# Kyo-suke-S/Depth_image_captioning_pub

Measured on AMD Instinct MI355X. Metric: images/sec (train, depth-soft, 224x224, seq-len 20), higher is better.
Workload: dtype f32; 1 GPU; depth-soft train step, synthetic RGB-D 224x224, batch 64/GPU, seq-len 20, V=10000, ResNet-152 (random init, batch-stat BN) + depth CNN + soft-attention LSTM; global_batch=64, batch_per_gpu=64, seq_len=20, vocab=10000, parallelism=dp1, resnet_conv_mode=f16x2, cross_step_resnet_overlap=True, resnet_forwards_in_flight=3, annotation_cells=49, ranks=1, collective=none (single rank)

## Files before the change

depth_image_captioning_pub_amd/csrc/api.hip:

```cpp
#include "dic.h"
#include "conv.h"
#include "nn_kernels.h"

#include <cstdio>

using namespace dic;

namespace dic { void resnet_fuse_bn_operand(int mask); void resnet_fuse_bn_halo(int on); void resnet_fuse_res_bn(int on); void depth_encoder_l1_sparse(int on); void bn_finalize_two_level_rows(int rows); void resnet_debug_fused_tail_bn(int on); void conv1_depth_debug_blocks(int n);
                void depth_encoder_f16x2(int on); }
#ifdef DIC_EXPERIMENTS
namespace dic { void decoder_debug_persistent(int on); void decoder_persist_debug_buffer(unsigned long long* p); void decoder_persist_debug_placement(int p);
                void resnet_debug_skip_bn_apply(int on); }
#endif

extern "C" {

int dic_version(void) { return DIC_ABI_VERSION; }
size_t dic_struct_bytes(int which) {
  switch (which) {
    case 0: return sizeof(dic_conv_bn_layer);
    case 1: return sizeof(dic_decoder_weights);
    case 2: return sizeof(dic_decoder_grads);
    case 3: return sizeof(dic_depth_encoder_weights);
    case 4: return sizeof(dic_depth_encoder_grads);
    case 5: return sizeof(dic_depth_bn_state);
    case 6: return sizeof(dic_nic_weights);
    case 7: return sizeof(dic_nic_grads);
    default: return 0;
  }
}
const char* dic_last_error(void) { return last_error(); }

int dic_gemm_f32(int M, int N, int K, const float* A, long long lda, int a_colk, const float* B, long long ldb,
                 int b_colk, float* C, long long ldc, const float* bias, int act, int accumulate, int splitk,
                 float* workspace, size_t workspace_bytes, int force_tile, void* stream) {
  GemmParams p{};
  p.M = M; p.N = N; p.K = K;
  p.A = a_colk ? op_colk(A, lda) : op_rowk(A, lda);
  p.B = b_colk ? op_colk(B, ldb) : op_rowk(B, ldb);
  p.ep = ep_store(C, ldc, bias, act);
  p.ep.accumulate = accumulate;
  p.splitk = splitk; p.ws = workspace;
  p.ablate = force_tile / 1000;
  force_tile %= 1000;
  DIC_REQUIRE(force_tile == 0 || force_tile == 64 || force_tile == 128, "force_tile must be 0, 64 or 128");
  if (splitk > 1)
    DIC_REQUIRE(workspace_bytes >= gemm_splitk_ws_bytes(M, N, splitk), "dic_gemm_f32: workspace too small");
  return gemm_launch(p, (hipStream_t)stream, force_tile);
}

int dic_conv2d_fwd(const float* x, int B, int H, int W, int C, int in_nchw, const float* w_ohwi, const float* bias,
                   int CO, int KH, int KW, int stride, int pad, float* y_nhwc, float* bn_partial, int* mtiles_out,
                   int force_tile, float* tail_ws, void* stream) {
  ConvDesc d{B, H, W, C, CO, KH, KW, stride, pad, in_nchw};
  return conv_fwd(x, d, w_ohwi, bias, y_nhwc, bn_partial, mtiles_out, (hipStream_t)stream, force_tile, tail_ws);
}

int dic_debug_force_staged_gemm(int on) {
  if (gemm_bf3_force_tile(on) == 0) return 0;
  if (on >= 100 && on <= 104) { dic::resnet_fuse_bn_operand(on == 104 ? -1 : on - 100); return 0; }
  if (on == 98 || on == 99) { dic::resnet_fuse_res_bn(on - 98); return 0; }
  if (on == 108 || on == 109) { dic::resnet_fuse_bn_halo(on - 108); return 0; }
  if (on == 182 || on == 183) { dic::bn_finalize_two_level_rows(on == 182 ? 512 : 1024); return 0; }
  if (on == 180 || on == 181) { dic::depth_encoder_l1_sparse(on - 180); return 0; }
  if (on == 116 || on == 117) { dic::depth_encoder_f16x2(on - 116); return 0; }
#ifdef DIC_EXPERIMENTS
  if (on == 140 || on == 141) { dic::decoder_debug_persistent(on - 140); return 0; }
  if (on == 142 || on == 143) { dic::decoder_persist_debug_placement(on - 142); return 0; }
  if (on >= 130 && on <= 134) { dic::conv1_depth_debug_blocks(256 * (on - 130)); return 0; }
  if (on >= 150 && on <= 153) { dic::resnet_debug_fused_tail_bn(on - 150); return 0; }
  if (on >= 124 && on <= 127) { dic::resnet_debug_skip_bn_apply(on == 125 ? 3 : on == 126 ? 2 : on == 127 ? 1 : 0); return 0; }
  if (on >= 0 && on <= 13) { gemm_force_v1(on); return 0; }
#endif
  DIC_REQUIRE(false, "debug switch: unknown code %d", on);
  return 0;
}
#ifdef DIC_EXPERIMENTS
int dic_debug_decoder_stamps(unsigned long long* dev_buf) { dic::decoder_persist_debug_buffer(dev_buf); return 0; }
#endif
int dic_debug_conv1_wgrad(const float* x, int B, int H, int W, const float* dy, float* dw, float* dbias, float* ws, float* cs_ws,
                          void* stream) {
  ConvDesc d{B, H, W, 1, 128, 7, 7, 3, 0, 0};
  return conv1_depth_wgrad(x, d, dy, dw, dbias, ws, cs_ws, (hipStream_t)stream);
}
int dic_debug_conv1_fwd(const float* x, int B, int H, int W, const float* w, const float* bias, float* y, float* partial,
                        void* stream) {
  ConvDesc d{B, H, W, 1, 128, 7, 7, 3, 0, 0};
  int rows = 0;
  return conv1_depth_fwd(x, d, w, bias, y, partial, &rows, (hipStream_t)stream);
}
int dic_debug_conv_bf3(const uint16_t* const x_planes[3], int B, int H, int W, int C, const uint16_t* const w_planes[3], int CO,
                       int k, int stride, int pad, float* y, float* bn_partial, int* mtiles_out, float* tail_ws, void* stream) {
  ConvDesc d{B, H, W, C, CO, k, k, stride, pad, 0};
  return conv_fwd_bf3(x_planes, d, w_planes, y, bn_partial, mtiles_out, tail_ws, (hipStream_t)stream, nullptr, nullptr, nullptr);
}
// ... 350 lines not shown
```

depth_image_captioning_pub_amd/csrc/conv.h:

```cpp
#pragma once
#include "gemm.h"

namespace dic {

struct ConvDesc {
  int B, H, W, C;
  int CO, KH, KW, stride, pad;
  int in_nchw;
  int OH() const { return (H + 2 * pad - KH) / stride + 1; }
  int OW() const { return (W + 2 * pad - KW) / stride + 1; }
  int M() const { return B * OH() * OW(); }
  int K() const { return KH * KW * C; }
  ConvGeom geom() const { return ConvGeom{H, W, C, OH(), OW(), KH, KW, stride, pad, in_nchw}; }
};

int conv_fwd(const float* x, const ConvDesc& d, const float* w_ohwi, const float* bias, float* y,
             float* bn_partial, int* mtiles_out, hipStream_t st, int force_tile = 0, float* tail_ws = nullptr);
int conv_mtiles(const ConvDesc& d, int force_tile = 0);

int conv_fwd_bf3(const unsigned short* const x_planes[3], const ConvDesc& d, const unsigned short* const w_planes[3],
                 float* y, float* bn_partial, int* mtiles_out, float* tail_ws, hipStream_t st,
                 const float* bias = nullptr, const BnFuseArgs* bn_fuse = nullptr, int* bn_fused = nullptr,
                 int act = 0 , int tail_ws_slabs = 256 ,
                 int fmt = 0 ,
                 float out_scale = 1.0f ,
                 const float* alpha_dev0 = nullptr, const float* alpha_dev1 = nullptr );
int conv1x1_fwd_bf3_bn(const float* raw, const float* scale, const float* shift, const float* res, int relu, float* act_out,
                       int M, int C, const unsigned short* const w_planes[3], int CO, float* y, float* bn_partial,
                       int* mtiles_out, float* tail_ws, int tail_ws_slabs, hipStream_t st, const BnFuseArgs* bn_fuse = nullptr,
                       int* bn_fused = nullptr, int fmt = 0, float out_scale = 1.0f,
                       unsigned* status = nullptr ,
                       const float* res_scale = nullptr, const float* res_shift = nullptr );
bool conv1x1_bf3_bn_eligible(const float* raw, int M, int C, int CO, float* tail_ws, int tail_ws_slabs, int fmt = 0);
int bf3_plan_route(int route, int fmt, const ConvDesc& d, int flags, int splitk, int tail_ws_slabs, const char** kernel, int out[6]);
int conv3x3_fwd_bf3_bn(const float* raw, const float* scale, const float* shift, int relu, const ConvDesc& d,
                       const unsigned short* const w_planes[3], float* y, float* bn_partial, int* mtiles_out, float* tail_ws,
                       int tail_ws_slabs, hipStream_t st, const BnFuseArgs* bn_fuse, int* bn_fused, int fmt, float out_scale, unsigned* status);
#ifdef DIC_EXPERIMENTS
bool conv1x1_astat_eligible(int M, int C, int CO);
int conv1x1_astat_bn(const float* raw, const float* scale, const float* shift, int relu, int M, int C, const unsigned short* const w_planes[3],
                     int CO, float* y, float* bn_partial, int* mtiles_out, hipStream_t st, float out_scale, unsigned* status = nullptr);
#endif
constexpr int kResnetTailSlabs = 1024;
size_t conv_wgrad_bf3_plane_elems(const ConvDesc& d, int which);
size_t conv_wgrad_bf3_ws_floats(const ConvDesc& d, int splitk);
int conv_wgrad_bf3(const float* x, const ConvDesc& d, const float* dy, float* dw_ohwi, int splitk,
                   unsigned short* const dyT[3], unsigned short* const pT[3], float* ws, hipStream_t st,
                   int fmt = 0, const float* dy_slot = nullptr );
size_t conv_stem_bf3_plane_elems(int B, int H, int W);
int conv_stem_pack_weights(const float* w_oihw, int CO, float* scratch_f32, unsigned short* const w_planes[3], hipStream_t st,
                           float f16_scale = 0.f );
int conv_stem_bf3(const float* imgs_nchw, int B, int H, int W, int CO, unsigned short* const x_planes[3],
                  const unsigned short* const w_planes[3], float* y, float* bn_partial, int* mtiles_out, hipStream_t st,
                  int fmt = 0, float out_scale = 1.0f, unsigned* status = nullptr );
int conv_dgrad_s1_bf3(const unsigned short* const dy_planes[3], const ConvDesc& d,
                      const unsigned short* const wflip_planes[3], float* dx, hipStream_t st, float* tail_ws = nullptr,
                      int tail_ws_slabs = 256, int fmt = 0, const float* alpha_dev0 = nullptr, const float* alpha_dev1 = nullptr);
int split_bf16x3(const float* x, long long n, unsigned short* hi, unsigned short* mid, unsigned short* lo, hipStream_t st);
int split_bf16x3_paired(const float* x, long long rows, int K, unsigned short* hi, unsigned short* mid,
                        unsigned short* lo, hipStream_t st);
int split_f16x2_paired(const float* x, long long rows, int K, float scale, unsigned short* h1, unsigned short* h2, hipStream_t st,
                       unsigned* status = nullptr );

int conv1_depth_fwd(const float* x, const ConvDesc& d, const float* w, const float* bias, float* y, float* bn_partial,
                    int* partial_rows, hipStream_t st);
int conv1_depth_fwd_blocks(const ConvDesc& d);
bool conv1_depth_supported(const ConvDesc& d);
size_t conv1_depth_wgrad_ws_floats(const ConvDesc& d);
struct BnBuf;
bool depth_layer1_sparse_supported(const ConvDesc& d);
size_t depth_layer1_sparse_ws_floats(const ConvDesc& d);
int conv1_depth_wgrad(const float* x, const ConvDesc& d, const float* dy, float* dw, float* dbias, float* ws, float* cs_ws,
                      hipStream_t st);
int depth_layer1_backward_sparse(const float* depth, const ConvDesc& d, const float* dpool, const unsigned char* idx, const float* xsel,
                                 const float* conv_w, const float* conv_b, const float* gamma, BnBuf bn, float* dgamma, float* dbeta,
                                 float* dW, float* db, float* bn_ws, float* ws, float* cs_ws, hipStream_t st);
int depth_prepare_weights(const float* w2, const float* w3, unsigned short* const w2_pl[3], unsigned short* const w2f_pl[3],
                          unsigned short* const w3_pl[3], unsigned short* const w3f_pl[3], const float* slots, hipStream_t st);
int conv_wgrad(const float* x, const ConvDesc& d, const float* dy, float* dw_ohwi, int splitk, float* ws,
               hipStream_t st);
int conv_dgrad_s1(const float* dy, const ConvDesc& d, const float* w_flip, float* dx, hipStream_t st);
int conv_flip_weights(const float* w_ohwi, const ConvDesc& d, float* w_flip, hipStream_t st);

}
```

depth_image_captioning_pub_amd/csrc/encoders.hip:

```cpp
#include "dic.h"
#include "conv.h"
#include "nn_kernels.h"
#include <algorithm>
#include <vector>

namespace dic {

struct DepthGeom {
  int B, H, W;
  int H1, W1, P1h, P1w, H2, W2, P2h, P2w;
  ConvDesc c1, c2, c3;
  long long M1, M2, M3;
};

static DepthGeom depth_geom(int B, int H, int W) {
  DepthGeom g{};
  g.B = B; g.H = H; g.W = W;
  g.c1 = ConvDesc{B, H, W, 1, 128, 7, 7, 3, 0, 1};
  g.H1 = g.c1.OH(); g.W1 = g.c1.OW();
  g.P1h = g.H1 / 3; g.P1w = g.W1 / 3;
  g.c2 = ConvDesc{B, g.P1h, g.P1w, 128, 512, 3, 3, 1, 0, 0};
  g.H2 = g.c2.OH(); g.W2 = g.c2.OW();
  g.P2h = g.H2 / 3; g.P2w = g.W2 / 3;
  g.c3 = ConvDesc{B, g.P2h, g.P2w, 512, 2048, 1, 1, 1, 0, 0};
// ... 224 lines not shown
                      (double)d.M(), kBnEps, kBnMomentum, fmt ? ws.status : nullptr};
  const int rc = conv1x1_fwd_bf3_bn(raw, in_bn.scale, in_bn.shift, res, 1, act_out, d.M(), d.C, wp, d.CO, y, train_bn ? ws.partial : nullptr,
                                    &mtiles, ws.tail, kResnetTailSlabs, st, (train_bn && g_fused_tail_bn) ? &fa : nullptr, &fused, fmt,
                                    fmt ? 1.0f / (kF16ActScale * L.w_scale) : 1.0f, fmt ? ws.status : nullptr,
                                    res_bn ? res_bn->scale : nullptr, res_bn ? res_bn->shift : nullptr);
  if (rc != DIC_OK) return rc;
  if (train_bn && fused) return DIC_OK;
  if (train_bn)
    return bn_finalize_train(ws.partial, mtiles, d.M(), d.CO, L.gamma, L.beta, L.running_mean, L.running_var, bn, ws.red, st,
                             fmt ? ws.status : nullptr);
  return bn_finalize_eval(d.CO, L.gamma, L.beta, L.running_mean, L.running_var, bn, st);
}

#ifdef DIC_EXPERIMENTS
static int conv_bn_bf3_astat(const float* raw, const BnBuf& in_bn, const ConvDesc& d, const dic_conv_bn_layer& L, float* y, const RnWs& ws,
                             int train_bn, hipStream_t st, const BnBuf& bn) {
  if (!(d.KH == 1 && d.KW == 1 && d.stride == 1 && d.pad == 0) || !conv1x1_astat_eligible(d.M(), d.C, d.CO)) return 1;
  int mtiles = 0;
  const unsigned short* wp[3] = {L.w_hi, L.w_mid, nullptr};
  DIC_TRY(conv1x1_astat_bn(raw, in_bn.scale, in_bn.shift, 1, d.M(), d.C, wp, d.CO, y, train_bn ? ws.partial : nullptr, &mtiles, st,
                           1.0f / (kF16ActScale * L.w_scale), ws.status));
  if (train_bn)
    return bn_finalize_train(ws.partial, mtiles, d.M(), d.CO, L.gamma, L.beta, L.running_mean, L.running_var, bn, ws.red, st, ws.status);
  return bn_finalize_eval(d.CO, L.gamma, L.beta, L.running_mean, L.running_var, bn, st);
}
#endif

static int g_fuse_bn_operand_switch = -1;
void resnet_fuse_bn_operand(int mask) { g_fuse_bn_operand_switch = mask < 0 ? -1 : (mask & 3); }
static int g_fuse_res_bn = 1;
void resnet_fuse_res_bn(int on) { g_fuse_res_bn = on; }
static int g_fuse_bn_halo = 1;
void resnet_fuse_bn_halo(int on) { g_fuse_bn_halo = on; }

static int conv_bn_bf3_halo_fused(const float* raw, const BnBuf& in_bn, const ConvDesc& d, const dic_conv_bn_layer& L, float* y, const RnWs& ws,
                                  int train_bn, hipStream_t st, const BnBuf& bn, int fmt) {
  if (!fmt || !g_fuse_bn_halo) return 1;
  int mtiles = 0, fused = 0;
  const unsigned short* wp[3] = {L.w_hi, L.w_mid, L.w_lo};
  const BnFuseArgs fa{L.gamma, L.beta, L.running_mean, L.running_var, bn.scale, bn.shift, bn.mean, bn.invstd,
                      (double)d.M(), kBnEps, kBnMomentum, ws.status};
  const int rc = conv3x3_fwd_bf3_bn(raw, in_bn.scale, in_bn.shift, 1, d, wp, y, train_bn ? ws.partial : nullptr, &mtiles, ws.tail, kResnetTailSlabs, st,
                                    (train_bn && g_fused_tail_bn) ? &fa : nullptr, &fused, fmt, 1.0f / (kF16ActScale * L.w_scale), ws.status);
  if (rc != DIC_OK) return rc;
  if (train_bn && fused) return DIC_OK;
  if (train_bn)
    return bn_finalize_train(ws.partial, mtiles, d.M(), d.CO, L.gamma, L.beta, L.running_mean, L.running_var, bn, ws.red, st, ws.status);
  return bn_finalize_eval(d.CO, L.gamma, L.beta, L.running_mean, L.running_var, bn, st);
}

static int resnet_fwd_bf3(const dic_conv_bn_layer* layers, const int* blocks, const float* imgs_nchw, int B, int train_bn,
                          float* features, const RnPlan& pl, const RnWs& ws, hipStream_t st, int pool_out, int fmt) {
  const int g_fuse_bn_operand = g_fuse_bn_operand_switch >= 0 ? g_fuse_bn_operand_switch : (fmt ? 1 : 3);
  unsigned* const guard = fmt ? ws.status : nullptr;
  size_t ci = 0;
  float *R2 = ws.act[0], *R3 = ws.act[1], *R1 = ws.act[2], *Cf = ws.act[3];
  float* const IN[2] = {ws.act[4], ws.act[5]};
  float* const X = ws.act[0];
  unsigned short* pset[3][3];
  for (int i = 0; i < 3; ++i)
    for (int j = 0; j < 3; ++j) pset[i][j] = (fmt && j == 2) ? nullptr : ws.planes[i][j];
  unsigned short* const* Xp = pset[0];
  unsigned short* const* P1 = pset[1];
  unsigned short* const* P2 = pset[2];
  {
    const RnConv& c = pl.convs[ci++];
    const dic_conv_bn_layer& L0 = layers[c.layer];
    const bool stem_f16 = fmt && L0.w_hi && L0.w_mid && !L0.w_lo && L0.w_scale > 0.f;
    if (g_strip_stem && L0.w_hi && L0.w_mid && (L0.w_lo || stem_f16) && c.d.H % 2 == 0 && c.d.W % 2 == 0) {
      int mtiles = 0;
      const unsigned short* wp[3] = {L0.w_hi, L0.w_mid, L0.w_lo};
      DIC_TRY(conv_stem_bf3(imgs_nchw, B, c.d.H, c.d.W, 64, ws.stem_planes, wp, R3, train_bn ? ws.partial : nullptr, &mtiles, st,
                            stem_f16 ? 1 : 0, stem_f16 ? 1.0f / (kF16ActScale * L0.w_scale) : 1.0f, guard));
      if (train_bn)
        DIC_TRY(bn_finalize_train(ws.partial, mtiles, c.d.M(), 64, L0.gamma, L0.beta, L0.running_mean, L0.running_var, ws.bn,
                                  ws.red, st, guard));
      else
        DIC_TRY(bn_finalize_eval(64, L0.gamma, L0.beta, L0.running_mean, L0.running_var, ws.bn, st));
    } else
    DIC_TRY(conv_bn(imgs_nchw, c.d, layers[c.layer], R3, ws.partial, ws.bn, ws.red, ws.tail, train_bn, st));
    DIC_TRY(bn_relu_maxpool(R3, B, c.d.OH(), c.d.OW(), 64, &ws.bn, 1, 3, 2, 1, nullptr, nullptr, st, Xp, guard));
  }
  for (int s = 0; s < 4; ++s) {
    bool pending = false;
    const float* pend_res = nullptr;
    const BnBuf* pend_res_bn = nullptr;
    const float* in32_carry = nullptr;
    for (int b = 0; b < blocks[s]; ++b) {
      const RnConv& c1 = pl.convs[ci++];
      const RnConv& c2 = pl.convs[ci++];
      const RnConv& c3 = pl.convs[ci++];
      const float* in32 = in32_carry;
      in32_carry = nullptr;
      if (pending) {
        float* in_b = IN[b & 1];
        int rc = conv_bn_bf3_fused(R3, ws.bn3, pend_res, in_b, c1.d, layers[c1.layer], R1, ws, train_bn, st, ws.bn, fmt, pend_res_bn);
        if (rc == 1) {
          DIC_BN_APPLY_PLANES_OUT(R3, pend_res, nullptr, in_b, Xp, c1.d.M(), c1.d.C, ws.bn3, 1, st, pend_res_bn, guard);
          rc = conv_bn_bf3(Xp, c1.d, layers[c1.layer], R1, ws, train_bn, st, nullptr, fmt);
        }
        DIC_TRY(rc);
        in32 = in_b;
      } else {
        DIC_TRY(conv_bn_bf3(Xp, c1.d, layers[c1.layer], R1, ws, train_bn, st, nullptr, fmt));
      }
      {
        int rc = conv_bn_bf3_halo_fused(R1, ws.bn, c2.d, layers[c2.layer], R2, ws, train_bn, st, ws.bn2, fmt);
        if (rc == 1) {
          DIC_BN_APPLY_PLANES(R1, nullptr, nullptr, nullptr, P1, c1.d.M(), c1.d.CO, ws.bn, 1, st, nullptr, guard);
          rc = conv_bn_bf3(P1, c2.d, layers[c2.layer], R2, ws, train_bn, st, &ws.bn2, fmt);
        }
        DIC_TRY(rc);
      }
      if (b == 0) {
// ... 234 lines not shown

int dic_depth_encoder_bwd_map(const dic_depth_encoder_weights* w, const float* depth, const float* d_feature_map, int B,
                              int H, int W, const dic_depth_encoder_grads* gr, void* workspace, size_t workspace_bytes,
                              void* stream) {
  return depth_encoder_bwd_impl(w, depth, d_feature_map, B, H, W, gr, workspace, workspace_bytes, stream, 0);
}

int dic_depth_encoder_inspect(const void* workspace, size_t workspace_bytes, int B, int H, int W, int which, void* out,
                              long long* n_out, void* stream) {
  DIC_REQUIRE(workspace && B > 0 && which >= 1 && which <= 5, "depth_encoder_inspect: bad arguments");
  const DepthGeom g = depth_geom(B, H, W);
  bool ov = false;
  DepthWs ws = depth_carve(const_cast<void*>(workspace), workspace_bytes, g, &ov);
  DIC_REQUIRE(!ov, "depth_encoder_inspect: workspace too small");
  const long long n = which <= 2 ? (long long)B * g.P1h * g.P1w * 128
                      : which <= 4 ? (long long)B * g.P2h * g.P2w * 512 : g.M3 * 2048;
  if (n_out) *n_out = n;
  if (!out) return DIC_OK;
  if (which == 5) return relu_mask_export(ws.x3, g.M3, 2048, ws.bn3, (unsigned char*)out, (hipStream_t)stream);
  const void* src = which == 1 ? (const void*)ws.y1p : which == 2 ? (const void*)ws.idx1 : which == 3 ? (const void*)ws.y2p
                                                                                                      : (const void*)ws.idx2;
  const size_t bytes = (size_t)n * ((which & 1) ? sizeof(float) : 1);
  DIC_CHECK_HIP(hipMemcpyAsync(out, src, bytes, hipMemcpyDeviceToDevice, (hipStream_t)stream));
  return DIC_OK;
}

int dic_resnet_pack_stem_weights(const float* w_oihw, float* scratch_f32, uint16_t* w_hi, uint16_t* w_mid, uint16_t* w_lo,
                                 void* stream) {
  DIC_REQUIRE(w_oihw && scratch_f32 && w_hi && w_mid && w_lo, "resnet_pack_stem_weights: null pointer");
  unsigned short* wp[3] = {w_hi, w_mid, w_lo};
  return conv_stem_pack_weights(w_oihw, 64, scratch_f32, wp, (hipStream_t)stream);
}

int dic_resnet_pack_stem_weights_f16x2(const float* w_oihw, float* scratch_f32, uint16_t* w_h1, uint16_t* w_h2, float w_scale, void* stream) {
  DIC_REQUIRE(w_oihw && scratch_f32 && w_h1 && w_h2 && w_scale > 0.f, "resnet_pack_stem_weights_f16x2: null pointer / scale");
  unsigned short* wp[3] = {w_h1, w_h2, nullptr};
  return conv_stem_pack_weights(w_oihw, 64, scratch_f32, wp, (hipStream_t)stream, w_scale);
}

int dic_resnet_num_layers(const int* blocks) {
  int n = 1;
  for (int s = 0; s < 4; ++s) n += 3 * blocks[s] + 1;
  return n;
}

size_t dic_resnet_workspace_bytes(int B, int H, int W, const int* blocks, int mode) {
  bool ov;
  return rn_carve(nullptr, 0, resnet_plan(B, H, W, blocks), mode, &ov).bytes;
}

static int resnet_fwd_impl(const dic_conv_bn_layer* layers, int n_layers, const int* blocks, const float* imgs_nchw, int B,
                           int H, int W, int train_bn, int mode, float* features, void* workspace, size_t workspace_bytes,
                           void* stream, int pool_out) {
  hipStream_t st = (hipStream_t)stream;
  DIC_REQUIRE(layers && blocks && imgs_nchw && features && workspace, "resnet_fwd: null pointer");
  DIC_REQUIRE(n_layers == dic_resnet_num_layers(blocks), "resnet_fwd: expected %d conv+bn layers, got %d",
              dic_resnet_num_layers(blocks), n_layers);
  DIC_REQUIRE(B > 0 && H >= 32 && W >= 32, "resnet_fwd: bad input size");
  const RnPlan pl = resnet_plan(B, H, W, blocks);
  bool ov = false;
  DIC_REQUIRE(mode >= 0 && mode <= 2, "resnet_fwd: mode must be 0 (exact-fp32 MFMA), 1 (bf16x3 split MFMA) or 2 (f16x2 split MFMA)");
  RnWs ws = rn_carve(workspace, workspace_bytes, pl, mode, &ov);
  DIC_REQUIRE(!ov, "resnet_fwd: workspace too small (%zu < %zu)", workspace_bytes, ws.bytes);
  DIC_TRY(clear_status(ws.status, st));
  if (mode >= 1) {
    for (int i = 1; i < n_layers; ++i) {
// ... 58 lines not shown
```

include/dic.h:

```cpp
#ifndef DIC_H_
#define DIC_H_
#include <stddef.h>
#include <stdint.h>

#ifdef __cplusplus
extern "C" {
#endif

#define DIC_L 196
#define DIC_D 2048
#define DIC_A 128
#define DIC_E 128
#define DIC_H 128

#define DIC_ABI_VERSION 200
int dic_version(void);
const char* dic_last_error(void);
size_t dic_struct_bytes(int which);

int dic_gemm_f32(int M, int N, int K, const float* A, long long lda, int a_colk, const float* B, long long ldb,
                 int b_colk, float* C, long long ldc, const float* bias, int act, int accumulate, int splitk,
                 float* workspace, size_t workspace_bytes, int force_tile, void* stream);

int dic_conv2d_fwd(const float* x, int B, int H, int W, int C, int in_nchw, const float* w_ohwi, const float* bias,
// ... 328 lines not shown
                     float out_scale, void* stream);
int dic_gemm_bf16x3(int M, int N, int K, const uint16_t* a_hi, const uint16_t* a_mid, const uint16_t* a_lo,
                    long long lda, const uint16_t* b_hi, const uint16_t* b_mid, const uint16_t* b_lo, long long ldb,
                    float* C, long long ldc, const float* bias, void* stream);

int dic_weight_standardize(const float* w, int O, int K, float eps, float* out, void* stream);
int dic_pad_nhwc(const float* x, int B, int H, int W, int C, int top, int left, int bottom, int right, float value,
                 float* out, void* stream);
int dic_maxpool_nhwc(const float* x, int B, int H, int W, int C, int k, int stride, float* out, void* stream);
size_t dic_groupnorm_workspace_bytes(int B, int groups);
int dic_groupnorm_nhwc(const float* x, int B, long long HW, int C, int groups, const float* gamma, const float* beta,
                       float eps, const float* residual, int relu, float* out, void* workspace, void* stream);
int dic_layernorm(const float* x, long long rows, int C, const float* gamma, const float* beta, float eps, float* out,
                  void* stream);
size_t dic_vit_attention_workspace_bytes(int B, int N, int heads);
int dic_vit_attention(const float* qkv, int B, int N, int heads, int head_dim, float* out, void* workspace,
                      size_t workspace_bytes, void* stream);
int dic_upsample2x_bilinear_nhwc(const float* x, int B, int H, int W, int C, float* out, void* stream);
int dic_add_act(const float* a, const float* b, long long n, long long period, int act, float* out, void* stream);
int dic_pointwise_dot(const float* x, long long rows, int C, const float* w, const float* bias, int relu, float* out,
                      void* stream);

int dic_normalize_images(const float* in, float* out, int B, int C, int H, int W, const float* mean3, const float* std3,
                         void* stream);
int dic_resize_bilinear(const float* in, int planes, int H, int W, int resize_short, int crop, float mul, float add,
                        float* out, void* stream);
int dic_depth_standardize(float* depth, int B, long long hw, void* stream);
int dic_bn_ema_update(float* running, const float* delta, long long n, float momentum, void* stream);
int dic_bn_ema_update_guarded(float* running, const float* delta, long long n, float momentum, const uint32_t* skip_if_raised,
                              void* stream);
int dic_gather_rows(const float* table, const int64_t* idx, int n, long long row_floats, float* out, void* stream);

int dic_debug_force_staged_gemm(int on);
int dic_debug_bn_finalize(const float* partial, int mtiles, long long count, int C, const float* gamma, const float* beta,
                          float* running_mean, float* running_var, float* scale, float* shift, float* mean, float* invstd, double* red,
                          size_t red_doubles, uint32_t* status, void* stream);
int dic_debug_bn_finalize_eval(int C, const float* gamma, const float* beta, const float* running_mean, const float* running_var,
                               float* scale, float* shift, float* mean, float* invstd, void* stream);
int dic_debug_bn_apply(const float* x, const float* residual, const uint16_t* const residual_planes[3], float* y, uint16_t* const planes[3],
                       long long rows, int C, const float* scale, const float* shift, const float* mean, const float* invstd, int relu,
                       const float* res_scale, const float* res_shift, const float* res_mean, const float* res_invstd, uint32_t* status,
                       void* stream);
int dic_debug_bn_relu_maxpool(const float* x, int B, int H, int W, int C, const float* scale, const float* shift, const float* mean,
                              const float* invstd, int relu, int k, int s, int p, float* y, unsigned char* idx, uint16_t* const planes[3],
                              uint32_t* status, float* xsel, void* stream);
int dic_debug_adaptive_avgpool(const float* x, int B, int H, int W, int C, const float* scale, const float* shift, const float* mean,
                               const float* invstd, int relu, int out, float* y, void* stream);
int dic_debug_adaptive_avgpool_bwd(const float* dy, int B, int H, int W, int C, int out, float* dx, void* stream);
int dic_debug_maxpool_relu_bwd(const float* dpool, const unsigned char* idx, const float* x, int B, int H, int W, int C, int k,
                               const float* scale, const float* shift, const float* mean, const float* invstd, float* dy, void* stream);
int dic_debug_relu_mask_bwd(float* dy, const float* x, long long rows, int C, const float* scale, const float* shift, const float* mean,
                            const float* invstd, void* stream);
int dic_debug_bn_backward_ws_floats(int C);
int dic_debug_bn_backward(float* dy_dx, const float* x, long long rows, int C, const float* gamma, const float* scale, const float* shift,
                          const float* mean, const float* invstd, float* dgamma, float* dbeta, float* ws, size_t ws_floats,
                          uint16_t* const dx_planes[3], uint32_t* f16_bound, float* f16_slot, void* stream);
int dic_debug_bn_pool_backward(const float* dpool, const unsigned char* idx, const float* x, int B, int H, int W, int C, int k,
                               const float* gamma, const float* scale, const float* shift, const float* mean, const float* invstd,
                               float* dgamma, float* dbeta, float* ws, size_t ws_floats, float* dy, uint16_t* const dy_planes[3],
                               uint32_t* f16_bound, float* f16_slot, void* stream);
int dic_debug_colsum_rows(const float* X, long long ld, long long rows, int C, float* out, float* ws, size_t ws_floats, void* stream);
int dic_debug_f16_scale_reset(uint32_t* bounds, int n, void* stream);
int dic_debug_f16_scale_from_absmax(const float* x, long long n, uint32_t* bound, float* slot, void* stream);
int dic_debug_f16_scale_finish(uint32_t* bound, float* slot, void* stream);
int dic_debug_conv_wgrad_sizes(int B, int H, int W, int C, int CO, int k, int stride, int pad, int splitk, size_t* dyT_elems, size_t* pT_elems,
                               size_t* ws_floats);
// ... 31 lines not shown
```

Baseline: 7540 images/s.

## Fuse ResNet stem conv with maxpool via pooled max/min and deferred BN

Adds a fused stem kernel that computes the 7x7 stride-2 conv with f16x2 MFMA per pooled tile, accumulates the BN statistics, and writes only the 3x3 maxpool max and min of the raw conv output instead of the full 112x112x64 map. A second pass applies BN+ReLU and chooses max or min according to the sign of the BN scale, which keeps the result exact. This removes the write and re-read of the large stem activation and the separate bn_relu_maxpool pass. In exchange, pooling windows overlap across tiles, so some conv outputs are recomputed at tile halos, and the new path is enabled by default.

```diff
diff --git a/depth_image_captioning_pub_amd/csrc/api.hip b/depth_image_captioning_pub_amd/csrc/api.hip
--- a/depth_image_captioning_pub_amd/csrc/api.hip
+++ b/depth_image_captioning_pub_amd/csrc/api.hip
@@ -6,7 +6,7 @@
 
 using namespace dic;
 
-namespace dic { void resnet_fuse_bn_operand(int mask); void resnet_fuse_bn_halo(int on); void resnet_fuse_res_bn(int on); void depth_encoder_l1_sparse(int on); void bn_finalize_two_level_rows(int rows); void resnet_debug_fused_tail_bn(int on); void conv1_depth_debug_blocks(int n);
+namespace dic { void resnet_fuse_bn_operand(int mask); void resnet_fuse_bn_halo(int on); void resnet_fuse_res_bn(int on); void resnet_stem_fused(int on); void depth_encoder_l1_sparse(int on); void bn_finalize_two_level_rows(int rows); void resnet_debug_fused_tail_bn(int on); void conv1_depth_debug_blocks(int n);
                 void depth_encoder_f16x2(int on); }
 #ifdef DIC_EXPERIMENTS
 namespace dic { void decoder_debug_persistent(int on); void decoder_persist_debug_buffer(unsigned long long* p); void decoder_persist_debug_placement(int p);
@@ -61,6 +61,7 @@
   if (on >= 100 && on <= 104) { dic::resnet_fuse_bn_operand(on == 104 ? -1 : on - 100); return 0; }
   if (on == 98 || on == 99) { dic::resnet_fuse_res_bn(on - 98); return 0; }
   if (on == 108 || on == 109) { dic::resnet_fuse_bn_halo(on - 108); return 0; }
+  if (on == 186 || on == 187) { dic::resnet_stem_fused(on - 186); return 0; }
   if (on == 182 || on == 183) { dic::bn_finalize_two_level_rows(on == 182 ? 512 : 1024); return 0; }
   if (on == 180 || on == 181) { dic::depth_encoder_l1_sparse(on - 180); return 0; }
   if (on == 116 || on == 117) { dic::depth_encoder_f16x2(on - 116); return 0; }
diff --git a/depth_image_captioning_pub_amd/csrc/conv.h b/depth_image_captioning_pub_amd/csrc/conv.h
--- a/depth_image_captioning_pub_amd/csrc/conv.h
+++ b/depth_image_captioning_pub_amd/csrc/conv.h
@@ -53,6 +53,12 @@
 int conv_stem_bf3(const float* imgs_nchw, int B, int H, int W, int CO, unsigned short* const x_planes[3],
                   const unsigned short* const w_planes[3], float* y, float* bn_partial, int* mtiles_out, hipStream_t st,
                   int fmt = 0, float out_scale = 1.0f, unsigned* status = nullptr );
+struct BnBuf;
+int conv_stem_pool_rows(int B, int H, int W);
+int conv_stem_pool_f16(const float* imgs_nchw, int B, int H, int W, const unsigned short* w_h1, const unsigned short* w_h2, float out_scale,
+                       float* pmax, float* pmin, float* bn_partial, unsigned* status, hipStream_t st);
+int stem_pool_bn_relu(const float* pmax, const float* pmin, long long rows, const BnBuf& bn, float* y, unsigned short* const planes[3],
+                      unsigned* status, hipStream_t st);
 int conv_dgrad_s1_bf3(const unsigned short* const dy_planes[3], const ConvDesc& d,
                       const unsigned short* const wflip_planes[3], float* dx, hipStream_t st, float* tail_ws = nullptr,
                       int tail_ws_slabs = 256, int fmt = 0, const float* alpha_dev0 = nullptr, const float* alpha_dev1 = nullptr);
@@ -67,7 +73,6 @@
 int conv1_depth_fwd_blocks(const ConvDesc& d);
 bool conv1_depth_supported(const ConvDesc& d);
 size_t conv1_depth_wgrad_ws_floats(const ConvDesc& d);
-struct BnBuf;
 bool depth_layer1_sparse_supported(const ConvDesc& d);
 size_t depth_layer1_sparse_ws_floats(const ConvDesc& d);
 int conv1_depth_wgrad(const float* x, const ConvDesc& d, const float* dy, float* dw, float* dbias, float* ws, float* cs_ws,
diff --git a/depth_image_captioning_pub_amd/csrc/encoders.hip b/depth_image_captioning_pub_amd/csrc/encoders.hip
--- a/depth_image_captioning_pub_amd/csrc/encoders.hip
+++ b/depth_image_captioning_pub_amd/csrc/encoders.hip
@@ -280,6 +280,27 @@
 void resnet_fuse_res_bn(int on) { g_fuse_res_bn = on; }
 static int g_fuse_bn_halo = 1;
 void resnet_fuse_bn_halo(int on) { g_fuse_bn_halo = on; }
+static int g_stem_fused = 1;
+void resnet_stem_fused(int on) { g_stem_fused = on; }
+
+static bool stem_fused_takes(int B, int H, int W) {
+  return g_stem_fused && H % 2 == 0 && W % 2 == 0 && H >= 6 && W >= 6 &&
+         conv_stem_pool_rows(B, H, W) <= (int)((long long)B * (H / 2) * (W / 2) / 32 + 4);
+}
+static int stem_fused_fwd(const float* imgs_nchw, int B, int H, int W, const dic_conv_bn_layer& L0, int train_bn, float* mm, float* partial,
+                          double* red, const BnBuf& bn, float* y, unsigned short* const planes[3], unsigned* guard, hipStream_t st) {
+  const int OH = H / 2, OW = W / 2, PH = (OH - 1) / 2 + 1, PW = (OW - 1) / 2 + 1;
+  const long long rows = (long long)B * PH * PW;
+  float *pmax = mm, *pmin = mm + rows * 64;
+  DIC_TRY(conv_stem_pool_f16(imgs_nchw, B, H, W, L0.w_hi, L0.w_mid, 1.0f / (kF16ActScale * L0.w_scale), pmax, pmin,
+                             train_bn ? partial : nullptr, guard, st));
+  if (train_bn)
+    DIC_TRY(bn_finalize_train(partial, conv_stem_pool_rows(B, H, W), (long long)B * OH * OW, 64, L0.gamma, L0.beta, L0.running_mean,
+                              L0.running_var, bn, red, st, guard));
+  else
+    DIC_TRY(bn_finalize_eval(64, L0.gamma, L0.beta, L0.running_mean, L0.running_var, bn, st));
+  return stem_pool_bn_relu(pmax, pmin, rows, bn, y, planes, guard, st);
+}
 
 static int conv_bn_bf3_halo_fused(const float* raw, const BnBuf& in_bn, const ConvDesc& d, const dic_conv_bn_layer& L, float* y, const RnWs& ws,
                                   int train_bn, hipStream_t st, const BnBuf& bn, int fmt) {
@@ -315,6 +336,9 @@
     const RnConv& c = pl.convs[ci++];
     const dic_conv_bn_layer& L0 = layers[c.layer];
     const bool stem_f16 = fmt && L0.w_hi && L0.w_mid && !L0.w_lo && L0.w_scale > 0.f;
+    if (stem_f16 && g_strip_stem && stem_fused_takes(B, c.d.H, c.d.W)) {
+      DIC_TRY(stem_fused_fwd(imgs_nchw, B, c.d.H, c.d.W, L0, train_bn, R3, ws.partial, ws.red, ws.bn, nullptr, Xp, guard, st));
+    } else {
     if (g_strip_stem && L0.w_hi && L0.w_mid && (L0.w_lo || stem_f16) && c.d.H % 2 == 0 && c.d.W % 2 == 0) {
       int mtiles = 0;
       const unsigned short* wp[3] = {L0.w_hi, L0.w_mid, L0.w_lo};
@@ -328,6 +352,7 @@
     } else
     DIC_TRY(conv_bn(imgs_nchw, c.d, layers[c.layer], R3, ws.partial, ws.bn, ws.red, ws.tail, train_bn, st));
     DIC_TRY(bn_relu_maxpool(R3, B, c.d.OH(), c.d.OW(), 64, &ws.bn, 1, 3, 2, 1, nullptr, nullptr, st, Xp, guard));
+    }
   }
   for (int s = 0; s < 4; ++s) {
     bool pending = false;
@@ -628,6 +653,50 @@
   return conv_stem_pack_weights(w_oihw, 64, scratch_f32, wp, (hipStream_t)stream);
 }
 
+static size_t stem_debug_carve(Carver& c, int B, int H, int W, unsigned short* planes[3], float** raw, float** partial, double** red, BnBuf* bn) {
+  const ConvDesc d{B, H, W, 3, 64, 7, 7, 2, 3, 1};
+  for (int j = 0; j < 2; ++j) planes[j] = c.take<unsigned short>(conv_stem_bf3_plane_elems(B, H, W));
+  planes[2] = nullptr;
+  *raw = c.take<float>((size_t)d.M() * 64 + 2 * 64 * 64);
+  *partial = c.take<float>((size_t)(d.M() / 32 + 4) * 2 * 64);
+  *red = c.take<double>(bn_finalize_ws_doubles(d.M() / 32 + 4, 64));
+  *bn = take_bn(c, 64);
+  return c.off;
+}
+int dic_debug_resnet_stem_ws_floats(int B, int H, int W) {
+  if (B < 1 || H < 2 || W < 2 || (long long)B * H * W > (1ll << 26)) return -1;
+  Carver c(nullptr, 0);
+  unsigned short* pl[3]; float *raw, *partial; double* red; BnBuf bn;
+  return (int)((stem_debug_carve(c, B, H, W, pl, &raw, &partial, &red, &bn) + 3) / 4);
+}
+int dic_debug_resnet_stem(const float* imgs_nchw, int B, int H, int W, const uint16_t* w_h1, const uint16_t* w_h2, float w_scale,
+                          const float* gamma, const float* beta, float* running_mean, float* running_var, int train_bn, float* y,
+                          float* ws, size_t ws_floats, uint32_t* status, void* stream) {
+  DIC_REQUIRE(imgs_nchw && w_h1 && w_h2 && gamma && beta && y && ws, "dic_debug_resnet_stem: null pointer");
+  DIC_REQUIRE(w_scale > 0.f && H % 2 == 0 && W % 2 == 0, "dic_debug_resnet_stem: w_scale=%g H=%d W=%d (positive scale, even image sizes)", w_scale, H, W);
+  DIC_REQUIRE(train_bn || (running_mean && running_var), "dic_debug_resnet_stem: eval mode needs the running statistics");
+  const int need = dic_debug_resnet_stem_ws_floats(B, H, W);
+  DIC_REQUIRE(need > 0 && ws_floats >= (size_t)need, "dic_debug_resnet_stem: workspace of %zu floats, %d needed", ws_floats, need);
+  hipStream_t st = (hipStream_t)stream;
+  Carver c(ws, ws_floats * sizeof(float));
+  unsigned short* pl[3]; float *raw, *partial; double* red; BnBuf bn;
+  stem_debug_carve(c, B, H, W, pl, &raw, &partial, &red, &bn);
+  dic_conv_bn_layer L0{};
+  L0.w_hi = const_cast<uint16_t*>(w_h1); L0.w_mid = const_cast<uint16_t*>(w_h2); L0.w_scale = w_scale;
+  L0.gamma = const_cast<float*>(gamma); L0.beta = const_cast<float*>(beta); L0.running_mean = running_mean; L0.running_var = running_var;
+  if (stem_fused_takes(B, H, W))
+    return stem_fused_fwd(imgs_nchw, B, H, W, L0, train_bn, raw, partial, red, bn, y, nullptr, status, st);
+  const int OH = H / 2, OW = W / 2;
+  int mtiles = 0;
+  const unsigned short* wp[3] = {w_h1, w_h2, nullptr};
+  DIC_TRY(conv_stem_bf3(imgs_nchw, B, H, W, 64, pl, wp, raw, train_bn ? partial : nullptr, &mtiles, st, 1, 1.0f / (kF16ActScale * w_scale), status));
+  if (train_bn)
+    DIC_TRY(bn_finalize_train(partial, mtiles, (long long)B * OH * OW, 64, gamma, beta, running_mean, running_var, bn, red, st, status));
+  else
+    DIC_TRY(bn_finalize_eval(64, gamma, beta, running_mean, running_var, bn, st));
+  return bn_relu_maxpool(raw, B, OH, OW, 64, &bn, 1, 3, 2, 1, y, nullptr, st, nullptr, status);
+}
+
 int dic_resnet_pack_stem_weights_f16x2(const float* w_oihw, float* scratch_f32, uint16_t* w_h1, uint16_t* w_h2, float w_scale, void* stream) {
   DIC_REQUIRE(w_oihw && scratch_f32 && w_h1 && w_h2 && w_scale > 0.f, "resnet_pack_stem_weights_f16x2: null pointer / scale");
   unsigned short* wp[3] = {w_h1, w_h2, nullptr};
diff --git a/depth_image_captioning_pub_amd/csrc/stem_fused.hip b/depth_image_captioning_pub_amd/csrc/stem_fused.hip
--- /dev/null
+++ b/depth_image_captioning_pub_amd/csrc/stem_fused.hip
@@ -0,0 +1,239 @@
+#include "conv.h"
+#include "nn_kernels.h"
+#include <algorithm>
+
+namespace dic {
+
+typedef _Float16 sp_f16x8 __attribute__((ext_vector_type(8)));
+typedef unsigned int sp_u32x4 __attribute__((ext_vector_type(4)));
+typedef float sp_f32x16 __attribute__((ext_vector_type(16)));
+
+constexpr int kSpT = 8;
+constexpr int kSpC = 2 * kSpT + 1;
+constexpr int kSpPix = kSpC * kSpC;
+constexpr int kSpMT = (kSpPix + 31) / 32;
+constexpr int kSpJ = kSpMT / 2;
+constexpr int kSpPR = 2 * (kSpC - 1) + 7;
+constexpr int kSpPC = 2 * (kSpC - 1) + 8;
+constexpr int kSpPU = (kSpPR * kSpPC + 255) / 256;
+constexpr int kSpPlaneB = kSpPR * kSpPC * 8;
+constexpr int kSpStageB = kSpPix * 64 * 4;
+static_assert(kSpMT % 2 == 0 && 2 * kSpPlaneB <= kSpStageB, "stem tile geometry");
+
+struct StemPoolParams {
+  const float* img;
+  const unsigned short *w1, *w2;
+  float *pmax, *pmin, *partial;
+  unsigned* status;
+  int B, H, W, OH, OW, PH, PW, ntH, ntW;
+  float alpha;
+};
+
+__global__ void __launch_bounds__(256, 2) stem_pool_f16_kernel(const StemPoolParams p) {
+  __shared__ __align__(16) unsigned char smem[kSpStageB];
+  __shared__ float red[4][2][64];
+  const int tid = threadIdx.x, lane = tid & 63, wave = tid >> 6, i31 = lane & 31, hh = lane >> 5;
+  int t = blockIdx.x;
+  const int tw = t % p.ntW; t /= p.ntW;
+  const int th = t % p.ntH;
+  const int b = t / p.ntH;
+  const int ph0 = th * kSpT, pw0 = tw * kSpT;
+  const int oh0 = 2 * ph0 - 1, ow0 = 2 * pw0 - 1;
+  const int ih0 = 2 * oh0 - 3, iw0 = 2 * ow0 - 3;
+  const int nh = wave & 1, mpar = wave >> 1;
+  const int n = nh * 32 + i31;
+
+  float pv[kSpPU][3];
+  const long long plane = (long long)p.H * p.W;
+#pragma unroll
+  for (int u = 0; u < kSpPU; ++u) {
+    const int i = min(tid + 256 * u, kSpPR * kSpPC - 1);
+    const int pr = i / kSpPC, pc = i - pr * kSpPC;
+    const int ih = ih0 + pr, iw = iw0 + pc;
+    const bool in = (unsigned)ih < (unsigned)p.H && (unsigned)iw < (unsigned)p.W;
+    const float* src = p.img + (long long)b * 3 * plane + (long long)min(max(ih, 0), p.H - 1) * p.W + min(max(iw, 0), p.W - 1);
+#pragma unroll
+    for (int c = 0; c < 3; ++c) {
+      const float x = src[c * plane];
+      pv[u][c] = in ? x : 0.f;
+    }
+  }
+  sp_u32x4 bf[14][2];
+#pragma unroll
+  for (int s = 0; s < 14; ++s) {
+    const long long off = plane_offset(n, (s >> 1) * 32 + ((s & 1) * 2 + hh) * 8, 7, 1);
+    bf[s][0] = *reinterpret_cast<const sp_u32x4*>(p.w1 + off);
+    bf[s][1] = *reinterpret_cast<const sp_u32x4*>(p.w2 + off);
+  }
+  bool bad = false;
+#pragma unroll
+  for (int u = 0; u < kSpPU; ++u) {
+    const int i = tid + 256 * u;
+    unsigned short a[4] = {0, 0, 0, 0}, m[4] = {0, 0, 0, 0};
+#pragma unroll
+    for (int c = 0; c < 3; ++c) {
+      bad |= f16x2_out_of_range(pv[u][c], kF16ActScale);
+      split2_f16(pv[u][c], kF16ActScale, a[c], m[c]);
+    }
+    if (i < kSpPR * kSpPC) {
+      *reinterpret_cast<uint2*>(smem + i * 8) = make_uint2((unsigned)a[0] | ((unsigned)a[1] << 16), (unsigned)a[2] | ((unsigned)a[3] << 16));
+      *reinterpret_cast<uint2*>(smem + kSpPlaneB + i * 8) = make_uint2((unsigned)m[0] | ((unsigned)m[1] << 16), (unsigned)m[2] | ((unsigned)m[3] << 16));
+    }
+  }
+  if (bad) f16x2_raise(p.status, 16u);
+  __syncthreads();
+
+  int abase[kSpJ];
+#pragma unroll
+  for (int j = 0; j < kSpJ; ++j) {
+    const int mc = min((mpar + 2 * j) * 32 + i31, kSpPix - 1);
+    const int r = mc / kSpC, c = mc - r * kSpC;
+    abase[j] = ((2 * r) * kSpPC + 2 * c + 2 * hh) * 8;
+  }
+  sp_f32x16 acc[kSpJ];
+#pragma unroll
+  for (int j = 0; j < kSpJ; ++j)
+#pragma unroll
+    for (int r = 0; r < 16; ++r) acc[j][r] = 0.f;
+#pragma unroll
+  for (int s = 0; s < 14; ++s) {
+    const int koff = ((s >> 1) * kSpPC + 4 * (s & 1)) * 8;
+    const sp_f16x8 b1 = __builtin_bit_cast(sp_f16x8, bf[s][0]), b2 = __builtin_bit_cast(sp_f16x8, bf[s][1]);
+#pragma unroll
+    for (int j = 0; j < kSpJ; ++j) {
+      const sp_f16x8 a1 = __builtin_bit_cast(sp_f16x8, *reinterpret_cast<const sp_u32x4*>(smem + abase[j] + koff));
+      const sp_f16x8 a2 = __builtin_bit_cast(sp_f16x8, *reinterpret_cast<const sp_u32x4*>(smem + kSpPlaneB + abase[j] + koff));
+      acc[j] = __builtin_amdgcn_mfma_f32_32x32x16_f16(a2, b1, acc[j], 0, 0, 0);
+      acc[j] = __builtin_amdgcn_mfma_f32_32x32x16_f16(a1, b2, acc[j], 0, 0, 0);
+      acc[j] = __builtin_amdgcn_mfma_f32_32x32x16_f16(a1, b1, acc[j], 0, 0, 0);
+    }
+  }
+  __syncthreads();
+
+  float* const stage = reinterpret_cast<float*>(smem);
+  {
+    float* const dst = stage + (mpar * 32 + 4 * hh) * 64 + n;
+#pragma unroll
+    for (int j = 0; j < kSpJ; ++j)
+#pragma unroll
+      for (int r = 0; r < 16; ++r) {
+        const int dm = 2 * j * 32 + (r & 3) + 8 * (r >> 2);
+        if (j < kSpJ - 1 || mpar * 32 + 4 * hh + dm < kSpPix) dst[dm * 64] = acc[j][r] * p.alpha;
+      }
+  }
+  __syncthreads();
+  const int ch = tid & 63, q = tid >> 6;
+  bool cv[5];
+  const float* colp[5];
+#pragma unroll
+  for (int k = 0; k < 5; ++k) cv[k] = (unsigned)(ow0 + 4 * q + k) < (unsigned)p.OW;
+#pragma unroll
+  for (int k = 0; k < 5; ++k) colp[k] = stage + (4 * q + (cv[k] ? k : (k >= 3 && cv[3]) ? 3 : 1)) * 64 + ch;
+  const bool st0 = pw0 + 2 * q < p.PW, st1 = pw0 + 2 * q + 1 < p.PW;
+  float* const omax = p.pmax + (((long long)b * p.PH + ph0) * p.PW + pw0 + 2 * q) * 64 + ch;
+  float* const omin = p.pmin + (((long long)b * p.PH + ph0) * p.PW + pw0 + 2 * q) * 64 + ch;
+  float cs = 0.f, cs2 = 0.f;
+  float hx0, hn0, hx1, hn1;
+  auto row = [&](int pr, float& x0, float& n0, float& x1, float& n1, bool sum) {
+    float x[5];
+#pragma unroll
+    for (int k = 0; k < 5; ++k) x[k] = colp[k][pr * kSpC * 64];
+    x0 = fmaxf(fmaxf(x[0], x[1]), x[2]); n0 = fminf(fminf(x[0], x[1]), x[2]);
+    x1 = fmaxf(fmaxf(x[2], x[3]), x[4]); n1 = fminf(fminf(x[2], x[3]), x[4]);
+    if (sum) {
+      const bool rv = (unsigned)(oh0 + pr) < (unsigned)p.OH;
+      float t[4];
+#pragma unroll
+      for (int k = 0; k < 4; ++k) t[k] = cv[k + 1] ? x[k + 1] : 0.f;
+      const float a1 = (t[0] + t[1]) + (t[2] + t[3]);
+      const float a2 = fmaf(t[0], t[0], t[1] * t[1]) + fmaf(t[2], t[2], t[3] * t[3]);
+      cs += rv ? a1 : 0.f;
+      cs2 += rv ? a2 : 0.f;
+    }
+  };
+  row(0, hx0, hn0, hx1, hn1, false);
+#pragma unroll
+  for (int py = 0; py < kSpT; ++py) {
+    float cx0, cn0, cx1, cn1, bx0, bn0, bx1, bn1;
+    row(2 * py + 1, cx0, cn0, cx1, cn1, true);
+    row(2 * py + 2, bx0, bn0, bx1, bn1, true);
+    const bool rt = (unsigned)(oh0 + 2 * py) < (unsigned)p.OH, rb = (unsigned)(oh0 + 2 * py + 2) < (unsigned)p.OH;
+    const float mx0 = fmaxf(fmaxf(rt ? hx0 : cx0, cx0), rb ? bx0 : cx0), mn0 = fminf(fminf(rt ? hn0 : cn0, cn0), rb ? bn0 : cn0);
+    const float mx1 = fmaxf(fmaxf(rt ? hx1 : cx1, cx1), rb ? bx1 : cx1), mn1 = fminf(fminf(rt ? hn1 : cn1, cn1), rb ? bn1 : cn1);
+    if (ph0 + py < p.PH) {
+      const long long o = (long long)py * p.PW * 64;
+      if (st0) { omax[o] = mx0; omin[o] = mn0; }
+      if (st1) { omax[o + 64] = mx1; omin[o + 64] = mn1; }
+    }
+    hx0 = bx0; hn0 = bn0; hx1 = bx1; hn1 = bn1;
+  }
+  red[q][0][ch] = cs;
+  red[q][1][ch] = cs2;
+  if (p.partial) {
+    __syncthreads();
+    if (tid < 128) p.partial[((long long)blockIdx.x * 2 + q) * 64 + ch] = (red[0][q][ch] + red[1][q][ch]) + (red[2][q][ch] + red[3][q][ch]);
+  }
+}
+
+static inline int sp_out(int n) { return (n - 1) / 2 + 1; }
+
+int conv_stem_pool_rows(int B, int H, int W) {
+  const int PH = sp_out(sp_out(H)), PW = sp_out(sp_out(W));
+  return B * ceil_div(PH, kSpT) * ceil_div(PW, kSpT);
+}
+
+int conv_stem_pool_f16(const float* imgs_nchw, int B, int H, int W, const unsigned short* w_h1, const unsigned short* w_h2, float out_scale,
+                       float* pmax, float* pmin, float* bn_partial, unsigned* status, hipStream_t st) {
+  DIC_REQUIRE(imgs_nchw && w_h1 && w_h2 && pmax && pmin, "conv_stem_pool_f16: null pointer");
+  DIC_REQUIRE(B >= 1 && H >= 2 && W >= 2 && H % 2 == 0 && W % 2 == 0, "conv_stem_pool_f16: B=%d H=%d W=%d (even image sizes)", B, H, W);
+  StemPoolParams p{};
+  p.img = imgs_nchw; p.w1 = w_h1; p.w2 = w_h2; p.pmax = pmax; p.pmin = pmin; p.partial = bn_partial; p.status = status;
+  p.B = B; p.H = H; p.W = W; p.OH = sp_out(H); p.OW = sp_out(W); p.PH = sp_out(p.OH); p.PW = sp_out(p.OW);
+  p.ntH = ceil_div(p.PH, kSpT); p.ntW = ceil_div(p.PW, kSpT);
+  p.alpha = out_scale;
+  DIC_REQUIRE((long long)B * p.ntH * p.ntW < (1ll << 31), "conv_stem_pool_f16: too many tiles");
+  hipLaunchKernelGGL(stem_pool_f16_kernel, dim3((unsigned)(B * p.ntH * p.ntW)), dim3(256), 0, st, p);
+  DIC_LAUNCH_CHECK();
+  return DIC_OK;
+}
+
+__global__ void __launch_bounds__(256) stem_pool_bn_relu_kernel(const float4* __restrict__ pmax, const float4* __restrict__ pmin, long long total,
+                                                                 BnBuf bn, float4* __restrict__ y, unsigned short* __restrict__ hi,
+                                                                 unsigned short* __restrict__ mid, unsigned* __restrict__ status) {
+  const long long stride = (long long)gridDim.x * 256;
+  for (long long i = (long long)blockIdx.x * 256 + threadIdx.x; i < total; i += stride) {
+    const long long row = i >> 4;
+    const int c4 = (int)(i & 15);
+    const float4 sc = *reinterpret_cast<const float4*>(bn.scale + c4 * 4), sh = *reinterpret_cast<const float4*>(bn.shift + c4 * 4);
+    const float4 mx = pmax[i], mn = pmin[i];
+    float4 v;
+    v.x = (sc.x >= 0.f ? mx.x : mn.x) * sc.x + sh.x; v.y = (sc.y >= 0.f ? mx.y : mn.y) * sc.y + sh.y;
+    v.z = (sc.z >= 0.f ? mx.z : mn.z) * sc.z + sh.z; v.w = (sc.w >= 0.f ? mx.w : mn.w) * sc.w + sh.w;
+    v.x = fmaxf(v.x, 0.f); v.y = fmaxf(v.y, 0.f); v.z = fmaxf(v.z, 0.f); v.w = fmaxf(v.w, 0.f);
+    if (y) y[i] = v;
+    if (hi) {
+      const long long off = plane_offset(row, c4 * 4, 2, 1);
+      unsigned short h[4], m[4];
+      if (f16x2_out_of_range(v.x, kF16ActScale) | f16x2_out_of_range(v.y, kF16ActScale) | f16x2_out_of_range(v.z, kF16ActScale) |
+          f16x2_out_of_range(v.w, kF16ActScale)) f16x2_raise(status, 2u);
+      split2_f16(v.x, kF16ActScale, h[0], m[0]); split2_f16(v.y, kF16ActScale, h[1], m[1]);
+      split2_f16(v.z, kF16ActScale, h[2], m[2]); split2_f16(v.w, kF16ActScale, h[3], m[3]);
+      *reinterpret_cast<uint2*>(hi + off) = make_uint2((unsigned)h[0] | ((unsigned)h[1] << 16), (unsigned)h[2] | ((unsigned)h[3] << 16));
+      *reinterpret_cast<uint2*>(mid + off) = make_uint2((unsigned)m[0] | ((unsigned)m[1] << 16), (unsigned)m[2] | ((unsigned)m[3] << 16));
+    }
+  }
+}
+
+int stem_pool_bn_relu(const float* pmax, const float* pmin, long long rows, const BnBuf& bn, float* y, unsigned short* const planes[3],
+                      unsigned* status, hipStream_t st) {
+  DIC_REQUIRE(pmax && pmin && rows >= 1 && (y || planes), "stem_pool_bn_relu: null pointer / no output");
+  DIC_REQUIRE(!planes || (planes[0] && planes[1] && !planes[2]), "stem_pool_bn_relu: f16x2 planes {h1, h2, NULL}");
+  const long long total = rows * 16;
+  hipLaunchKernelGGL(stem_pool_bn_relu_kernel, dim3((unsigned)std::min<long long>((total + 255) / 256, 8192)), dim3(256), 0, st,
+                     reinterpret_cast<const float4*>(pmax), reinterpret_cast<const float4*>(pmin), total, bn, reinterpret_cast<float4*>(y),
+                     planes ? planes[0] : nullptr, planes ? planes[1] : nullptr, status);
+  DIC_LAUNCH_CHECK();
+  return DIC_OK;
+}
+
+}
diff --git a/include/dic.h b/include/dic.h
--- a/include/dic.h
+++ b/include/dic.h
@@ -384,6 +384,10 @@
 int dic_gather_rows(const float* table, const int64_t* idx, int n, long long row_floats, float* out, void* stream);
 
 int dic_debug_force_staged_gemm(int on);
+int dic_debug_resnet_stem_ws_floats(int B, int H, int W);
+int dic_debug_resnet_stem(const float* imgs_nchw, int B, int H, int W, const uint16_t* w_h1, const uint16_t* w_h2, float w_scale,
+                          const float* gamma, const float* beta, float* running_mean, float* running_var, int train_bn, float* y,
+                          float* ws, size_t ws_floats, uint32_t* status, void* stream);
 int dic_debug_bn_finalize(const float* partial, int mtiles, long long count, int C, const float* gamma, const float* beta,
                           float* running_mean, float* running_var, float* scale, float* shift, float* mean, float* invstd, double* red,
                           size_t red_doubles, uint32_t* status, void* stream);
```

Measured after the change: 7423 images/s. 1.5% lower.
